# dojo-sim/ContactImplicitMPC.jl

Hardware: AMD Instinct MI355X
Metric: MPC steps/s (quadruped, H=40, fp64) (higher is better)
Workload: dtype f64

## Files before the change

contactimplicitmpc/jl_amd/csrc/cimpc_host.cpp:

```cpp
#include <hip/hip_runtime.h>

#include <algorithm>
#include <chrono>
#include <cmath>
#include <cstdio>
#include <cstdlib>
#include <cstring>
#include <string>
#include <vector>

#include "cimpc_internal.h"
#include "lin_table.h"
#include "model_table.h"
#include "newton_state.h"
#include "schedule_plan.h"

using namespace cimpc;

namespace {

thread_local std::string g_create_error;

enum ProfClass { PC_IP = 0, PC_KKT = 1, PC_RESID = 2, PC_OTHER = 3, PC_ASYNC = 4, PC_COUNT = 5 };

struct ProfRec {
    hipEvent_t a, b;
    int cls;
};

}

struct RoundStreams {
    hipStream_t st = nullptr;
    hipStream_t st_kkt = nullptr;
    hipEvent_t ev_join = nullptr;
    hipEvent_t ev_start = nullptr;
};

struct Knobs {
    SchedulePolicy sched{};
    bool async_debug = false;
    double watchdog_s = 30.0;
    bool debug_rounds = false;
    bool generic_static = false;
    KktPolicy kkt{};
    int kkt_tw_nb = 0;
    int kkt_tw_spins = 0;
    int banded_form = 0;

    static int env_int(const char* name, int dflt) { const char* v = getenv(name); return v ? atoi(v) : dflt; }
    void read_environment() {
        sched.async_mode = env_int("CIMPC_ASYNC", sched.async_mode);
        sched.async_tail = env_int("CIMPC_ASYNC_TAIL", sched.async_tail);
        sched.spec_first = env_int("CIMPC_SPEC_FIRST", sched.spec_first);
        sched.iter_cap = std::max(1, env_int("CIMPC_ITER_CAP", sched.iter_cap));
        async_debug = getenv("CIMPC_ASYNC_DEBUG") != nullptr;
        if (const char* v = getenv("CIMPC_ASYNC_WATCHDOG_S")) watchdog_s = atof(v);
        debug_rounds = getenv("CIMPC_DEBUG_ROUNDS") != nullptr;
        sched.tail_div = env_int("CIMPC_TAIL_DIV", sched.tail_div);
// ... 277 lines not shown
        if (h->d_mix_ws) return CIMPC_OK;
        if (dev_alloc(h, &h->d_mix_ws, kkt_mixed_workspace_doubles(h->S)) != CIMPC_OK) return CIMPC_ERR_HIP;
        return dev_alloc(h, &h->d_mix_nfb, 1);
    }
    const bool cf = h->kb == KktBackend::CfCondensed || h->kb == KktBackend::CfBanded;
    if (cf && !h->d_cf_ws && dev_alloc(h, &h->d_cf_ws, cf_reduce_doubles(h->S)) != CIMPC_OK) return CIMPC_ERR_HIP;
    if (h->kb == KktBackend::CfCondensed) return CIMPC_OK;
    const size_t need = cf ? kkt_dense_workspace_doubles(cf_shadow(h->S), true) : kkt_dense_workspace_doubles(h->S, h->kb == KktBackend::Banded);
    if (h->d_dense_ws && h->dense_ws_doubles >= need) return CIMPC_OK;
    h->d_dense_ws = nullptr;
    h->dense_ws_doubles = need;
    return dev_alloc(h, &h->d_dense_ws, need);
}

static KktForm plan_kkt_stage(cimpc_ctx* h, const KktSite& site) {
    const KktForm f = choose_kkt_form(h->kp, h->kc, h->kb, site);
    if (two_ended(f)) h->n_kkt_twisted++;
    return f;
}
static int run_kkt_stage(cimpc_ctx* h, const NewtonDev& Sk, const KktArgs& K, const KktSite& site, const int* list, int n, const int* n_dev, hipStream_t st) {
    return launch_kkt_stage(Sk, K, h->kb, plan_kkt_stage(h, site), list, n, n_dev, KktWorkspace{h->d_dense_ws, h->d_cf_ws, h->d_mix_ws, h->d_mix_nfb}, st);
}

int read_stats(cimpc_ctx* h, long long out[4]) {
    std::vector<long long> v((size_t)h->dm.B * 4);
    HIP_TRY(h, hipMemcpy(v.data(), h->S.stats, v.size() * sizeof(long long), hipMemcpyDeviceToHost));
    out[0] = out[1] = out[2] = out[3] = 0;
    for (size_t b = 0; b < (size_t)h->dm.B; ++b)
        for (int k = 0; k < 4; ++k) out[k] += v[b * 4 + k];
    return CIMPC_OK;
}

int drain_pending(cimpc_ctx* h) {
    if (!h->advance_pending) return CIMPC_OK;
    HIP_TRY(h, hipStreamSynchronize(h->stream));
    h->advance_pending = false;
    return CIMPC_OK;
}

int check_ready(cimpc_ctx* h, bool need_newton) {
    if (!h) return CIMPC_ERR_INVALID;
    if (h->n_knots_set != h->dm.H_ref)
        return fail(h, CIMPC_ERR_STATE, "set_linearization has not been called for every knot");
    if (!h->window_set) return fail(h, CIMPC_ERR_STATE, "set_window has not been called");
    if (need_newton) {
        if (!h->objective_set) return fail(h, CIMPC_ERR_STATE, "set_objective has not been called");
        if (!h->reference_set) return fail(h, CIMPC_ERR_STATE, "set_reference has not been called");
    }
    return CIMPC_OK;
}

}

extern "C" {

// ... 183 lines not shown
            g_create_error = "mapped counter allocation failed"; cimpc_destroy(h); return CIMPC_ERR_HIP;
        }
        h->h_twfail[0] = 0;
        S.kkt_tw_fail = dv;
    }
    if (hipHostMalloc((void**)&h->h_ring, RING_ALLOC_INTS * sizeof(int), hipHostMallocMapped) != hipSuccess ||
        hipHostGetDevicePointer((void**)&h->h_ring_dev, h->h_ring, 0) != hipSuccess) {
        g_create_error = "ring allocation failed"; cimpc_destroy(h); return CIMPC_ERR_HIP;
    }
    if (h->sched.async_on) {
        const size_t K = d.H_ref;
        if (dev_alloc(h, &h->a_items, K * h->a_cap) != CIMPC_OK || dev_alloc(h, &h->a_jobs, h->a_rq_cap + h->a_kq_cap) != CIMPC_OK ||
            dev_alloc(h, &h->a_ctrl, async_ctl(K).ints) != CIMPC_OK || dev_alloc(h, &h->a_evals, B) != CIMPC_OK) {
            g_create_error = h->err; cimpc_destroy(h); return CIMPC_ERR_HIP;
        }
        if (h->kn.async_debug && dev_alloc(h, &h->a_dbg, 16) != CIMPC_OK) { g_create_error = h->err; cimpc_destroy(h); return CIMPC_ERR_HIP; }
        h->async_dirty = true;
    }
    {
        RoundStreams& r = h->rs;
        if (hipStreamCreateWithFlags(&r.st, hipStreamNonBlocking) != hipSuccess ||
            hipStreamCreateWithFlags(&r.st_kkt, hipStreamNonBlocking) != hipSuccess ||
            hipEventCreateWithFlags(&r.ev_join, hipEventDisableTiming) != hipSuccess ||
            hipEventCreateWithFlags(&r.ev_start, hipEventDisableTiming) != hipSuccess) {
            g_create_error = "stream creation failed"; cimpc_destroy(h); return CIMPC_ERR_HIP;
        }
    }
    *out = h;
    return CIMPC_OK;
}

int cimpc_destroy(cimpc_handle h) {
    if (!h) return CIMPC_ERR_INVALID;
    (void)hipSetDevice(h->device);
    if (h->stream) (void)hipStreamSynchronize(h->stream);
    for (auto& r : h->prof_recs) { (void)hipEventDestroy(r.a); (void)hipEventDestroy(r.b); }
    for (auto e : h->ev_pool) (void)hipEventDestroy(e);
    for (void* p : h->allocs) (void)hipFree(p);
    if (h->h_counters) (void)hipHostFree(h->h_counters);
    if (h->h_ring) (void)hipHostFree(h->h_ring);
    if (h->h_qin) (void)hipHostFree(h->h_qin);
    if (h->h_result) (void)hipHostFree(h->h_result);
    if (h->h_stage) (void)hipHostFree(h->h_stage);
    if (h->h_twfail) (void)hipHostFree(h->h_twfail);
    {
        RoundStreams& r = h->rs;
        if (r.st) { (void)hipStreamSynchronize(r.st); (void)hipStreamDestroy(r.st); }
        if (r.st_kkt) { (void)hipStreamSynchronize(r.st_kkt); (void)hipStreamDestroy(r.st_kkt); }
        if (r.ev_join) (void)hipEventDestroy(r.ev_join);
        if (r.ev_start) (void)hipEventDestroy(r.ev_start);
    }
    if (h->own_stream && h->stream) (void)hipStreamDestroy(h->stream);
    delete h;
    return CIMPC_OK;
}

int cimpc_set_stream(cimpc_handle h, void* hip_stream) {
    if (!h) return CIMPC_ERR_INVALID;
    (void)hipStreamSynchronize(h->stream);
    h->advance_pending = false;
    if (h->own_stream && h->stream) (void)hipStreamDestroy(h->stream);
    h->stream = static_cast<hipStream_t>(hip_stream);
    h->own_stream = false;
    h->external_stream = true;
    return CIMPC_OK;
}

int cimpc_synchronize(cimpc_handle h) {
    if (!h) return CIMPC_ERR_INVALID;
    HIP_TRY(h, hipStreamSynchronize(h->stream));
    return CIMPC_OK;
}

// ... 390 lines not shown
}

NewtonDev launch_view(const cimpc_ctx* h, int parity) {
    NewtonDev Sk = h->S;
    Sk.b0 = 0; Sk.nb_launch = h->dm.B;
    Sk.counters = round_counter_block(h->d_ring, parity);
    Sk.counters_next = round_counter_block(h->d_ring, parity ^ 1);
    Sk.host_flag = ring_slot(h->h_ring_dev, parity);
    Sk.WQ = h->Q; Sk.WQ.par = parity;
    return Sk;
}
void wire_async_queues(const cimpc_ctx* h, NewtonDev& Sk) {
    const AsyncCtl L = async_ctl(h->Q.K);
    int* const c = h->a_ctrl;
    Sk.WQ.items = h->a_items; Sk.WQ.cap = (int)h->a_cap; Sk.WQ.count = c + L.count; Sk.WQ.head = c + L.head;
    AsyncQ& A = Sk.A;
    A.on = 1;
    A.rq_items = h->a_jobs; A.rq_head = c + L.rq_head; A.rq_tail = c + L.rq_tail;
    A.kq_items = h->a_jobs + h->a_rq_cap; A.kq_head = c + L.kq_head; A.kq_tail = c + L.kq_tail;
    A.n_done = c + L.n_done; A.epoch = c + L.epoch; A.evals_left = h->a_evals;
    A.abort_flag = ring_abort_word((volatile int*)h->h_ring_dev);
}

int finish_results(cimpc_ctx* h, hipStream_t st) {
    if (launch_dz_commit(h->S, st) != CIMPC_OK) return fail(h, CIMPC_ERR_HIP, "sensitivity flush launch failed");
    if (int rf = launch_solve_finish(h->S, h->d_result, st); rf != CIMPC_OK) return fail(h, rf, "result kernel launch failed");
    HIP_TRY(h, hipMemcpyAsync(h->h_result, h->d_result, result_doubles(h->dm.B, h->dm.nu) * sizeof(double), hipMemcpyDeviceToHost, st));
    return CIMPC_OK;
}
void publish_stats(cimpc_ctx* h, long long rounds) {
    const double* r = h->h_result;
    cimpc_stats& s = h->last_stats;
    s.sweeps = (long long)r[RESULT_SWEEPS]; s.ip_solves = (long long)r[RESULT_IP_SOLVES];
    s.ip_iters = (long long)r[RESULT_IP_ITERS]; s.ip_failures = (long long)r[RESULT_IP_FAILURES];
    s.rounds = rounds; s.newton_iters = (long long)r[RESULT_NEWTON_SUM];
}

int print_async_debug(cimpc_ctx* h) {
    long long dv[16];
    HIP_TRY(h, hipMemcpy(dv, h->a_dbg, sizeof(dv), hipMemcpyDeviceToHost));
    fprintf(stderr, "[cimpc async] WG-ms: other %.2f kkt %.2f resid %.2f ip %.2f | jobs: kkt %lld resid %lld serve %lld | grid %d service %d | group-trips %.2fM active %.1f%% | group-ms pop %.1f fence %.1f | pop: cas %lld spins %lld claim-ms %.1f wait-ms %.1f\n",
            dv[0] * 1e-5, dv[1] * 1e-5, dv[2] * 1e-5, dv[3] * 1e-5, dv[9], dv[10], dv[11], h->sched.async_grid, h->sched.async_service, dv[5] * 1e-6, dv[5] ? 100.0 * dv[4] / dv[5] : 0.0, dv[6] * 1e-5, dv[7] * 1e-5, dv[12], dv[13], dv[14] * 1e-5, dv[15] * 1e-5);
    return CIMPC_OK;
}
void print_queued_problems(cimpc_ctx* h, const SolveRun& run, long long r, int par, long long hint) {
    std::vector<int> qc((size_t)h->Q.K * QPAD);
    (void)hipStreamSynchronize(run.sb.st); (void)hipStreamSynchronize(run.sb.st_kkt);
    if (hipMemcpy(qc.data(), h->Q.count + (size_t)par * h->Q.K * QPAD, qc.size() * sizeof(int), hipMemcpyDeviceToHost) != hipSuccess) return;
    long long tot = 0;
    for (int k = 0; k < h->Q.K; ++k) tot += qc[(size_t)k * QPAD];
    fprintf(stderr, "[cimpc round %lld] sweep launch: %lld problems queued (host hint %lld)\n", r, tot, hint);
}

int run_async(cimpc_ctx* h, SolveRun& run, bool from_reset, long long rounds_before) {
    NewtonDev& S = h->S;
    IpQueues LQ = h->Q; LQ.par = (int)(rounds_before & 1);
    hipStream_t st = run.sb.st;
    if (h->async_dirty) {
        HIP_TRY(h, hipMemsetAsync(h->a_items, 0xFF, (size_t)h->Q.K * h->a_cap * sizeof(int), st));
        HIP_TRY(h, hipMemsetAsync(h->a_jobs, 0xFF, (h->a_rq_cap + h->a_kq_cap) * sizeof(int), st));
        h->async_dirty = false;
    }
    HIP_TRY(h, hipMemsetAsync(h->a_ctrl, 0, async_ctl(h->Q.K).ints * sizeof(int), st));
    volatile int* abort_word = ring_abort_word((volatile int*)h->h_ring);
    *abort_word = 0;
    NewtonDev Sk = launch_view(h, 0);
    if (!from_reset) Sk.spec_all = h->sched.spec_tail;
    wire_async_queues(h, Sk);
    AsyncQ& A = Sk.A;
    A.n_service = from_reset ? h->sched.async_service : h->sched.tail_service;
    A.idle_sleep = async_idle_sleep; A.idle_spins = async_idle_spins; A.wake_fan = async_wake_fan;
    A.dbg = h->a_dbg; A.B = h->dm.B;
    if (h->a_dbg) HIP_TRY(h, hipMemsetAsync(h->a_dbg, 0, 16 * sizeof(long long), st));
    const KktSite site{.kind = from_reset ? KktSite::Persistent : KktSite::HybridTail, .tw_off = *(volatile int*)h->h_twfail != run.tw_fail0,
                       .B = h->dm.B, .async_tail = h->sched.async_tail, .waves = std::min(h->sched.waves, 4)};
    A.kkt_tw = plan_kkt_stage(h, site) == KktForm::AsyncTwoJob ? 1 : 0;
    S.kkt_tw_epoch += h->nt.max_iter + 2;
    prof_begin(h, PC_OTHER, st);
    int rc2 = from_reset ? launch_reset(Sk, run.q0_dev, run.q1_dev, run.warm_start, st) : launch_async_handoff(Sk, LQ, st);
    prof_end(h, st);
    if (rc2 != CIMPC_OK) return fail(h, rc2, "reset / hand-off launch failed");
    IpParams p = make_ip_params(h, S.cand, 0, round_counter(h->d_ring, RC_PARKED), nullptr);
    if (S.dtn != nullptr) { p.nu = S.nu_cand; p.dtn = S.dtn; }
    p.Q = Sk.WQ;
    p.iter_cap = h->ip.max_iter + 1;
    p.A = A;
    long long solved_before = 0;
    if (h->prof_on && !from_reset) { long long sv[4]; if (int rs = read_stats(h, sv); rs != CIMPC_OK) return rs; solved_before = sv[1]; }
    prof_begin(h, PC_ASYNC, st);
    rc2 = launch_newton_async(&h->dm, p, Sk, std::min(h->sched.waves, 4), from_reset ? h->sched.async_grid : h->sched.tail_grid, st);
    prof_end(h, st);
    if (rc2 != CIMPC_OK) return fail(h, rc2, "asynchronous newton launch failed");
    if (int rf = finish_results(h, st); rf != CIMPC_OK) return rf;
    const bool budget = has_time_budget(h);
    bool timed_out = false; long long polls = 0;
    const auto tw = std::chrono::steady_clock::now();
    while (hipStreamQuery(st) == hipErrorNotReady) {
        const bool over = budget && over_budget(h, run);
        timed_out = !over && (++polls & 0x3FF) == 0 && std::chrono::duration<double>(std::chrono::steady_clock::now() - tw).count() > h->kn.watchdog_s;
        if (over || timed_out) { *abort_word = 1; h->async_dirty = true; break; }
    }
    HIP_TRY(h, hipStreamSynchronize(st));
    note_tw_fallbacks(h);
    if (timed_out) return fail(h, CIMPC_ERR_HIP, "asynchronous solve: watchdog expired (no completion within CIMPC_ASYNC_WATCHDOG_S)");
    if (h->a_dbg) { if (int rd = print_async_debug(h); rd != CIMPC_OK) return rd; }
    publish_stats(h, rounds_before + 1);
    h->prof_ip_problems += solved_before;
    h->prof_async_problems += h->last_stats.ip_solves - solved_before;
    if (from_reset) h->prof_kkt_systems += h->last_stats.newton_iters;
    return CIMPC_OK;
}

int launch_round(cimpc_ctx* h, SolveRun& run, long long r, bool blind) {
    const RoundStreams& sb = run.sb; const RoundCounts& last = run.last;
    const int par = (int)(r & 1);
    h->S.kkt_tw_epoch += 1;
    const bool tw_off = note_tw_fallbacks(h) != run.tw_fail0;
    NewtonDev Sk = launch_view(h, par);
    Sk.A.n_done = run.hybrid ? h->a_ctrl + async_ctl(h->Q.K).n_done : nullptr;
    Sk.round_stamp = (int)(r + 1);
    const bool kkt = (r > 0) && (blind || last.kkt > 0);
    const int n_kkt = blind ? h->dm.B : last.kkt;
    const int* n_kkt_dev = blind ? round_counter(Sk.counters_next, RC_KKT) : nullptr;
    if (kkt) {
        const bool ov = h->kp.kkt_overlap;
        const KktSite site{.kind = ov ? KktSite::Overlapped : KktSite::Round, .n_kkt = n_kkt, .blind = blind,
                           .sweep_problems = (long long)last.new_slots * h->dm.H, .tw_off = tw_off, .B = h->dm.B};
        hipStream_t kst = ov ? sb.st_kkt : sb.st;
        if (!ov) Sk.kkt_same_round = 1;
// ... 20 lines not shown
    if (rr != CIMPC_OK) return fail(h, rr, "residual launch failed");
    return CIMPC_OK;
}

}

int cimpc_newton_solve_dev(cimpc_handle h, const double* q0_dev, const double* q1_dev, int warm_start) {
    int rc = check_ready(h, true);
    if (rc != CIMPC_OK) return rc;
    if (!q0_dev || !q1_dev) return fail(h, CIMPC_ERR_INVALID, "null argument");
    HIP_TRY(h, hipSetDevice(h->device));
    if (int sy = sync_dz_stores(h, 1); sy != CIMPC_OK) return sy;
    h->dz_producer = 1;
    const int B = h->dm.B;
    SolveRun run{q0_dev, q1_dev, warm_start, {}, *(volatile int*)h->h_twfail, false, h->rs, RoundCounts{B, 0, B, B, 0, 0}};
    h->twfail_seen = run.tw_fail0;
    run.t0 = std::chrono::steady_clock::now();
    RoundStreams& sb = run.sb;
    if (h->external_stream) sb.st = h->stream;
    else {
        HIP_TRY(h, hipEventRecord(sb.ev_start, h->stream));
        HIP_TRY(h, hipStreamWaitEvent(sb.st, sb.ev_start, 0));
    }
    HIP_TRY(h, hipMemsetAsync(h->S.stats, 0, (size_t)B * 4 * sizeof(long long), sb.st));
    if ((rc = ensure_kkt_ws(h)) != CIMPC_OK) return rc;
    const SolvePath path = choose_solve_path(h->sched, h->kb);
    if (path == SolvePath::Persistent) return run_async(h, run, true, 0);
    run.hybrid = path == SolvePath::Hybrid;
    const int round_limit = max_rounds(h->kn.sched, h->nt.max_iter, h->ip.max_iter);
    long long launched = 0, completed = 0;
    const bool ahead = round_ahead(h->sched, h->kb, warm_start != 0, has_time_budget(h));
    HIP_TRY(h, hipMemsetAsync(h->Q.count, 0, h->ctl_ints * sizeof(int), sb.st));
    if (run.hybrid) HIP_TRY(h, hipMemsetAsync(h->a_ctrl + async_ctl(h->Q.K).jobs, 0, ASYNC_JOB_INTS * sizeof(int), sb.st));
    for (int slot = 0; slot < RING_SLOTS_COUNT; ++slot) ring_slot((volatile int*)h->h_ring, slot)[RING_STAMP] = 0;
    prof_begin(h, PC_OTHER, sb.st);
    rc = launch_reset(launch_view(h, 0), q0_dev, q1_dev, warm_start, sb.st);
    prof_end(h, sb.st);
    if (rc != CIMPC_OK) return fail(h, rc, "reset launch failed");
    while (true) {
        if (completed >= round_limit) {
            (void)hipStreamSynchronize(sb.st); (void)hipStreamSynchronize(sb.st_kkt);
            return fail(h, CIMPC_ERR_STATE, "newton_solve: round limit reached with unfinished rollouts");
        }
        while (launched <= completed + (ahead ? 1 : 0)) {
            rc = launch_round(h, run, launched, launched > completed);
            if (rc != CIMPC_OK) return rc;
            ++launched;
        }
        {
            volatile int* hm = ring_slot((volatile int*)h->h_ring, completed);
            const int want = (int)(completed + 1);
            long long spins = 0;
            while (hm[RING_STAMP] != want) {
                if ((++spins & 0xFFFFF) == 0 && hipStreamQuery(sb.st) != hipErrorNotReady && hm[RING_STAMP] != want)
                    return fail(h, CIMPC_ERR_HIP, "round finished without publishing its counters");
            }
        }
        const RoundCounts& last = run.last = read_round_counts(h->h_ring, completed);
        if (h->kn.debug_rounds) fprintf(stderr, "[cimpc round %lld] t %.3f ms: next sweep %d rollouts (%d evaluation slots), next kkt %d, parked %d, finished %d\n", completed,
                                        1e3 * elapsed_s(run), last.sweep, last.slots, last.kkt, last.parked, last.finished);
        h->prof_kkt_systems += last.kkt;
        ++completed;
        if ((last.sweep == 0 && last.kkt == 0) || over_budget(h, run)) break;
        if (run.hybrid && hand_over(h->sched, B - last.finished)) {
            HIP_TRY(h, hipStreamSynchronize(sb.st));
            HIP_TRY(h, hipStreamSynchronize(sb.st_kkt));
            return run_async(h, run, false, completed);
        }
    }
    HIP_TRY(h, hipStreamSynchronize(sb.st_kkt));
    if (int rf = finish_results(h, sb.st); rf != CIMPC_OK) return rf;
    HIP_TRY(h, hipStreamSynchronize(sb.st));
    publish_stats(h, completed);
    h->prof_ip_problems += h->last_stats.ip_solves;
    return CIMPC_OK;
}

int cimpc_newton_solve(cimpc_handle h, const double* q0, const double* q1, int warm_start,
                       double* u1, int* newton_iters, double* r_norm) {
    if (!h || !q0 || !q1) return fail(h, CIMPC_ERR_INVALID, "null argument");
    const size_t ne = (size_t)h->dm.B * h->dm.nq;
    HIP_TRY(h, hipSetDevice(h->device));
    std::memcpy(h->h_qin, q0, ne * sizeof(double));
    std::memcpy(h->h_qin + ne, q1, ne * sizeof(double));
    HIP_TRY(h, hipMemcpyAsync(h->d_q0, h->h_qin, 2 * ne * sizeof(double), hipMemcpyHostToDevice, h->stream));
    int rc = cimpc_newton_solve_dev(h, h->d_q0, h->d_q1, warm_start);
    if (rc != CIMPC_OK) return rc;
    const int nu = h->dm.nu;
    for (int b = 0; b < h->dm.B; ++b) {
        const double* o = h->h_result + result_u1(b, nu);
        if (u1) std::memcpy(u1 + (size_t)b * nu, o, nu * sizeof(double));
        if (newton_iters) newton_iters[b] = (int)o[record_iters(nu)];
        if (r_norm) r_norm[b] = o[record_r_norm(nu)] / (double)h->N;
    }
// ... 323 lines not shown
```

contactimplicitmpc/jl_amd/csrc/newton_impl.h:

```cpp
#pragma once
#include "lane_group.h"
#include "newton_state.h"

namespace cimpc {

struct BlockSync { static __device__ __forceinline__ void sync() { __syncthreads(); } };
struct WaveSync {
    static __device__ __forceinline__ void sync() {
        __builtin_amdgcn_fence(__ATOMIC_SEQ_CST, "workgroup");
        __builtin_amdgcn_wave_barrier();
    }
};

__device__ __forceinline__ void theta_update(const NewtonDev& S, const TrajDev& T, int b, int i,
                                             int tid, int nthreads) {
    const cimpc_dims& m = S.dm;
    double* th = T.th + ((size_t)b * m.H + i) * S.nth;
    const double* q = T.q + ((size_t)b * (m.H + 2) + i) * m.nq;
    const double* u = T.u + ((size_t)b * m.H + i) * m.nu;
    const double* w = T.w + ((size_t)b * m.H + i) * m.nw;
    for (int k = tid; k < 2 * m.nq; k += nthreads) th[k] = q[k];
    for (int k = tid; k < m.nu; k += nthreads) th[2 * m.nq + k] = u[k];
    for (int k = tid; k < m.nw; k += nthreads) th[2 * m.nq + m.nu + k] = w[k];
}
// ... 573 lines not shown
        }
        return;
    }
    const double alpha = ls_alpha(iter);
    if (act == 1) {
        if (iter <= 6) accept_candidate<BlockSync>(S, sb0 + it0 + slot, b, tid, nt);
        else apply_step<BlockSync>(S, S.traj, S.nu, (size_t)b, b, alpha, tid, nt);
    }
    RPROF(6)
    {
        double* rr = S.res + (size_t)b * S.N;
        const double* r = S.res_cand + (sb0 + it0 + slot) * S.N;
        for (int e = tid; e < S.N; e += nt) rr[e] = r[e];
    }
    RPROF(7)
    {
        const int blk = S.nths * S.nd, ita = it0 + slot;
        double* good = S.dz_good + (size_t)b * H * blk;
        {
        if constexpr (SPLIT == 2) {
            resolve_eff(slot, eff);
            __syncthreads();
        }
        bool lazy_commit = false;
        if constexpr (!ASYNC) lazy_commit = S.good_src != nullptr && use_eff;
        if (lazy_commit) {
            const int* ef = eff + (SPLIT ? 0 : slot * EFF_H);
            for (int i = tid; i < H; i += nt) S.good_src[(size_t)b * H + i] = ef[i];
        } else if (use_eff && (blk & 1) == 0) {
            const int* ef = eff + (SPLIT ? 0 : slot * EFF_H);
            const int hb = blk / 2;
            constexpr int UN = 13;
            for (int e0 = tid; e0 < H * hb; e0 += UN * nt) {
                typedef double v2d __attribute__((ext_vector_type(2)));
                v2d v[UN]; int dst[UN];
                static_for<0, UN>([&](auto jc) {
                    constexpr int j = decltype(jc)::value;
                    const int e = e0 + j * nt, ec = e < H * hb ? e : 0, i = ec / hb, s_ = ef[i];
                    dst[j] = (e < H * hb && s_ >= 0) ? i * blk + 2 * (ec - i * hb) : -1;
                    v[j] = reinterpret_cast<const v2d*>(S.dz + ((sb0 + (s_ >= 0 ? s_ : 0)) * H + i) * (size_t)blk)[ec - i * hb];
                });
                static_for<0, UN>([&](auto jc) {
                    constexpr int j = decltype(jc)::value;
                    if (dst[j] >= 0) *reinterpret_cast<v2d*>(good + dst[j]) = v[j];
                });
            }
        } else {
            for (int e = tid; e < H * blk; e += nt) {
// ... 1396 lines not shown
```

contactimplicitmpc/jl_amd/csrc/newton_kernels.hip:

```cpp
#include <cstdlib>
#ifdef CIMPC_KKT_PROF
#define CIMPC_KKT_WPROF
#endif
#include "newton_impl.h"
#include "model_table.h"

namespace cimpc {

__global__ __launch_bounds__(256) void reset_kernel(NewtonDev S, const double* q0,
                                                    const double* q1, int warm) {
    const cimpc_dims& m = S.dm;
    const int b = blockIdx.x + S.b0, tid = threadIdx.x, nt = blockDim.x;
    const int H = m.H;
    const size_t oq = (size_t)b * (H + 2) * m.nq;
    const size_t sb0 = (size_t)b * CS;
    if (!warm) {
        for (int k = tid; k < H * S.nd; k += nt) {
            S.nu[(size_t)b * H * S.nd + k] = 0.0;
        }
        copy_n(S.traj.q + oq, S.ref.q + oq, (H + 2) * m.nq, tid, nt);
        copy_n(S.traj.u + (size_t)b * H * m.nu, S.ref.u + (size_t)b * H * m.nu, H * m.nu, tid, nt);
        copy_n(S.traj.w + (size_t)b * H * m.nw, S.ref.w + (size_t)b * H * m.nw, H * m.nw, tid, nt);
        copy_n(S.traj.g + (size_t)b * H * m.nc, S.ref.g + (size_t)b * H * m.nc, H * m.nc, tid, nt);
        copy_n(S.traj.b + (size_t)b * H * m.nb, S.ref.b + (size_t)b * H * m.nb, H * m.nb, tid, nt);
        copy_n(S.traj.th + (size_t)b * H * S.nth, S.ref.th + (size_t)b * H * S.nth, H * S.nth, tid, nt);
    }
    __syncthreads();
    for (int k = tid; k < m.nq; k += nt) {
        S.traj.q[oq + k] = q0[(size_t)b * m.nq + k];
        S.traj.q[oq + m.nq + k] = q1[(size_t)b * m.nq + k];
    }
    __syncthreads();
    theta_update(S, S.traj, b, 0, tid, nt);
    if (H > 1) theta_update(S, S.traj, b, 1, tid, nt);
    __syncthreads();
    copy_n(S.cand.q + sb0 * (H + 2) * m.nq, S.traj.q + oq, (H + 2) * m.nq, tid, nt);
// ... 190 lines not shown
    KktArgs F = K0; F.only_flag = flag;
    rc = launch_kkt_condensed(S, F, KktForm::PerRollout, false, nullptr, S.nb_launch, nullptr, s);
    if (rc != CIMPC_OK) return rc;
    return hipGetLastError() == hipSuccess ? CIMPC_OK : CIMPC_ERR_HIP;
}

#ifdef CIMPC_RESID_PROF
extern "C" int cimpc_debug_resid_prof(unsigned long long* out32) {
    unsigned long long z[64] = {0};
    if (hipMemcpyFromSymbol(out32, HIP_SYMBOL(cimpc::g_resid_prof), sizeof(z)) != hipSuccess) return -1;
    return hipMemcpyToSymbol(HIP_SYMBOL(cimpc::g_resid_prof), z, sizeof(z)) == hipSuccess ? 0 : -1;
}
#endif
__global__ __launch_bounds__(64) void enqueue_all_kernel(NewtonDev S) {
    const int b = blockIdx.x + S.b0;
    enqueue_eval(S, (size_t)b * CS, b, S.WQ.par, threadIdx.x, 64, b - S.b0);
    if (threadIdx.x == 0) S.cur_slot[b] = 0;
    for (int k = threadIdx.x; k < S.dm.H; k += 64) S.pflag[(size_t)b * CS * S.dm.H + k] = 0;
}
int launch_enqueue_all(const NewtonDev& S, hipStream_t s) {
    hipLaunchKernelGGL(enqueue_all_kernel, dim3(S.nb_launch), dim3(64), 0, s, S);
    return hipGetLastError() == hipSuccess ? CIMPC_OK : CIMPC_ERR_HIP;
}
__global__ __launch_bounds__(64) void async_handoff_kernel(NewtonDev S, IpQueues LQ) {
    const int i = blockIdx.x, tid = threadIdx.x;
    if (i < S.WQ.K) {
        const int n = *qcount(LQ, LQ.par, i);
        const int* src = LQ.items + ((size_t)LQ.par * LQ.K + i) * LQ.cap;
        int* dst = S.WQ.items + (size_t)i * S.WQ.cap;
        for (int k = tid; k < n; k += 64) dst[k] = src[k];
        if (tid == 0) *qcount(S.WQ, 0, i) = n;
    }
    if (i < S.dm.B && tid == 0) {
        const int b = i, stage = S.stage[b];
        if (stage == STAGE_DONE) {
            atomicAdd(S.A.n_done, 1);
        } else if (stage == STAGE_KKT) {
            push_kkt_job(S.A, b);
        } else {
            const size_t sb0 = (size_t)b * CS;
            int n = 0;
            for (int c = 0; c < CS; ++c) n += (S.need_sweep[sb0 + c] != 0 && S.WQ.done_count[sb0 + c] < S.dm.H);
            S.A.evals_left[b] = n;
        }
    }
}
int launch_async_handoff(const NewtonDev& S, const IpQueues& LQ, hipStream_t s) {
    const int grid = S.dm.B > S.WQ.K ? S.dm.B : S.WQ.K;
    hipLaunchKernelGGL(async_handoff_kernel, dim3(grid), dim3(64), 0, s, S, LQ);
    return hipGetLastError() == hipSuccess ? CIMPC_OK : CIMPC_ERR_HIP;
}
__global__ __launch_bounds__(64) void mpc_advance_kernel(NewtonDev S, int* window, const double* stride, int H_ref) {
    const cimpc_dims& m = S.dm;
    const int b = blockIdx.x, c = threadIdx.x, H = m.H, nq = m.nq, nth = S.nth;
    auto rot = [&](double* a, int rows, int n) {
        if (c >= n) return;
        const double first = a[c];
        for (int t = 0; t + 1 < rows; ++t) a[(size_t)t * n + c] = a[(size_t)(t + 1) * n + c];
        a[(size_t)(rows - 1) * n + c] = first;
    };
    double* q = S.ref.q + (size_t)b * (H + 2) * nq;
    double* th = S.ref.th + (size_t)b * H * nth;
    rot(q, H + 2, nq);
    rot(S.ref.u + (size_t)b * H * m.nu, H, m.nu);
    rot(S.ref.w + (size_t)b * H * m.nw, H, m.nw);
    rot(S.ref.g + (size_t)b * H * m.nc, H, m.nc);
    rot(S.ref.b + (size_t)b * H * m.nb, H, m.nb);
    rot(th, H, nth);
    __syncthreads();
    if (c < nq) {
        q[(size_t)H * nq + c] = q[c] + stride[c];
        q[(size_t)(H + 1) * nq + c] = q[nq + c] + stride[c];
// ... 51 lines not shown
    hipLaunchKernelGGL(mpc_advance_kernel, dim3(S.dm.B), dim3(64), 0, s, S, window, stride, H_ref);
    return hipGetLastError() == hipSuccess ? CIMPC_OK : CIMPC_ERR_HIP;
}
__global__ __launch_bounds__(128) void dz_rekey_kernel(double* step_base, size_t stride_b, size_t stride_i, double* knot,
                                                       const int* window, int H, int K, int blk, int dir) {
    const int b = (int)blockIdx.x / H, i = (int)blockIdx.x - b * H;
    const int* w = window + (size_t)b * (H + 2);
    const int t = w[i];
    if (dir == 0)
        for (int j = i + 1; j < H; ++j) if (w[j] == t) return;
    double* st = step_base + (size_t)b * stride_b + (size_t)i * stride_i;
    double* kn = knot + ((size_t)b * K + t) * (size_t)blk;
    const double* src = dir == 0 ? st : kn;
    double* dst = dir == 0 ? kn : st;
    for (int e = (int)threadIdx.x; e < blk; e += (int)blockDim.x) dst[e] = src[e];
}
int launch_dz_rekey(const NewtonDev& S, double* knot, const int* window, int which, int dir, hipStream_t s) {
    const size_t blk = (size_t)S.nths * S.nd, H = S.dm.H;
    double* base = which == 0 ? S.dz_good : S.dz;
    const size_t stride_b = which == 0 ? H * blk : (size_t)CS * H * blk;
    hipLaunchKernelGGL(dz_rekey_kernel, dim3(S.dm.B * S.dm.H), dim3(128), 0, s, base, stride_b, blk, knot, window, S.dm.H, S.dm.H_ref, (int)blk, dir);
    return hipGetLastError() == hipSuccess ? CIMPC_OK : CIMPC_ERR_HIP;
}
int launch_reset(const NewtonDev& S, const double* q0, const double* q1, int warm, hipStream_t s) {
    hipLaunchKernelGGL(reset_kernel, dim3(S.nb_launch), dim3(256), 0, s, S, q0, q1, warm);
    return hipGetLastError() == hipSuccess ? CIMPC_OK : CIMPC_ERR_HIP;
}
template <int NQ, int NU, bool CF>
static int launch_resid_m(const NewtonDev& S, hipStream_t s, int n_slots, int phase) {
    const size_t lds2 = (size_t)2 * CIMPC_RESID_THREADS * sizeof(double);
    if (n_slots == -1) {
        const size_t lds1 = (size_t)(CS * 256 + S.N) * sizeof(double);
        if (lds1 <= 64 * 1024) {
            if (phase == 1) return CIMPC_OK;
            hipLaunchKernelGGL((resid_decide_kernel<NQ, NU, CF, true>), dim3(S.nb_launch), dim3(CIMPC_RESID_THREADS), lds1, s, S);
            return hipGetLastError() == hipSuccess ? CIMPC_OK : CIMPC_ERR_HIP;
        }
    }
    const int* list = (n_slots >= 0 && S.slot_list != nullptr) ? S.slot_list + (size_t)S.WQ.par * S.dm.B * CS : nullptr;
    const int grid = list != nullptr ? n_slots : S.nb_launch * CS;
    const size_t lds = (size_t)(256 + (S.N <= SLOT_ABS_MAX ? S.N : 0)) * sizeof(double);
    if (grid > 0 && phase != 2) hipLaunchKernelGGL((resid_slot_kernel<NQ, NU, CF>), dim3(grid), dim3(CIMPC_SLOT_THREADS), lds, s, S, list);
    if (phase != 1) hipLaunchKernelGGL((resid_decide_kernel<NQ, NU, CF, false>), dim3(S.nb_launch), dim3(CIMPC_RESID_THREADS), lds2, s, S);
    return hipGetLastError() == hipSuccess ? CIMPC_OK : CIMPC_ERR_HIP;
}
template <int NQ, int NU>
static int launch_resid_t(const NewtonDev& S, hipStream_t s, int n_slots, int phase) {
    return S.dm.mode == CIMPC_MODE_CONFIGURATIONFORCE ? launch_resid_m<NQ, NU, true>(S, s, n_slots, phase) : launch_resid_m<NQ, NU, false>(S, s, n_slots, phase);
// ... 214 lines not shown
```

contactimplicitmpc/jl_amd/csrc/newton_state.h:

```cpp
#pragma once
#include "cimpc_internal.h"
#include "kkt_plan.h"

namespace cimpc {
constexpr int NLOG = 16;

enum Stage : int { STAGE_DONE = 0, STAGE_INIT = 1, STAGE_LS0 = 2, STAGE_KKT = 3, STAGE_LS1 = 4, STAGE_LS2 = 5, STAGE_LS7 = 6, STAGE_LS3 = 7 };
constexpr int CS = 7;

struct TrajDev {
    double* q;
    double* u;
    double* w;
    double* g;
    double* b;
    double* th;
};

struct NewtonDev {
    cimpc_dims dm;
    int b0;
    int nb_launch;
    int kkt_same_round;
    int nd, nr, nth, nths, N;
// ... 41 lines not shown
    const double* Rinv;
    const double* Cg;
    const double* Cb;
    const double* V;
    const double* q_target;
    const double* v_target;
    double* kkt_ws;
    double* kkt_tw_xch;
    int* kkt_tw_flags;
    int kkt_tw_epoch;
    int kkt_tw_spins;
    int* kkt_tw_fail;
    int kkt_tw_nb;
    double r_tol, beta_init, kappa;
    int max_iter;
    double* nlog;
    int spec_first;
    int spec_mid;
    int spec_all;
};

bool newton_async_available(const cimpc_dims* dm);
int launch_newton_async(const cimpc_dims* dm, const IpParams& p, const NewtonDev& S, int waves, int grid, hipStream_t s);
int launch_async_handoff(const NewtonDev& S, const IpQueues& lockstep_next, hipStream_t s);
int launch_mpc_advance(const NewtonDev& S, int* window, const double* stride, int H_ref, hipStream_t s);
struct GaitDev {
    const double *q, *u, *w, *g, *b, *th;
    const double* stride;
    int* phase;
    int H_ref;
};
int launch_gait_window(const NewtonDev& S, const GaitDev& G, int* window, int advance, hipStream_t s);
int launch_reset(const NewtonDev& nd, const double* q0, const double* q1, int warm, hipStream_t s);
int launch_dz_commit(const NewtonDev& nd, hipStream_t s);
int launch_dz_rekey(const NewtonDev& nd, double* knot, const int* window, int which, int dir, hipStream_t s);
int launch_resid_decide(const NewtonDev& nd, hipStream_t s, int n_slots = -1, int phase = 0);
int launch_enqueue_all(const NewtonDev& nd, hipStream_t s);
struct KktArgs {
    const double* r;
    double* delta;
    const double* beta;
    double beta_scalar;
    const int* stage;
    int finish;
    const double* dz_override;
    const int* only_flag;
};
inline KktArgs kkt_newton_args(const NewtonDev& S) { return KktArgs{S.res, S.delta, S.beta, 0.0, S.stage, 1, nullptr, nullptr}; }
inline KktArgs kkt_raw_args(const double* r, double beta, double* delta) { return KktArgs{r, delta, nullptr, beta, nullptr, 0, nullptr, nullptr}; }
struct KktWorkspace { double* dense; double* cf; double* mix; int* mix_nfb; };
int launch_kkt_stage(const NewtonDev& S, const KktArgs& K, KktBackend be, KktForm f, const int* list, int n, const int* n_dev,
                     const KktWorkspace& W, hipStream_t s);
bool kkt_condensed_available(const NewtonDev& nd);
bool kkt_mfma_available(const NewtonDev& nd);
bool kkt_packed_available(const NewtonDev& nd);
bool kkt_twisted_available(const NewtonDev& nd);
// ... 15 lines not shown
```

contactimplicitmpc/jl_amd/csrc/round_protocol.h:

```cpp
#pragma once
#include <stddef.h>

#if defined(__HIPCC__)
#define ROUND_HD __host__ __device__ __forceinline__
#else
#define ROUND_HD inline
#endif

namespace cimpc {

constexpr int QPAD = 32;
constexpr int CPAD = 32;

enum RoundCounter : int {
    RC_SWEEP = 0,
    RC_KKT = 1,
    RC_PARKED = 2,
    RC_DRAINED = 3,
    RC_SLOTS = 4,
    RC_NEW_SLOTS = 5,
    RC_TICKET = 7,
};
constexpr int ROUND_COUNTERS = 8;
constexpr int ROUND_COUNTER_INTS = ROUND_COUNTERS * CPAD;
// ... 29 lines not shown
ROUND_HD constexpr int epoch_ip(int bucket) { return bucket * EPOCH_STRIDE; }
ROUND_HD constexpr int epoch_job(int bucket) { return (EPOCH_BUCKETS + bucket) * EPOCH_STRIDE; }
ROUND_HD constexpr int epoch_any_job() { return 2 * EPOCH_BUCKETS * EPOCH_STRIDE; }

constexpr int KJOB_SHIFT = 24, KJOB_MASK = (1 << KJOB_SHIFT) - 1;
enum KktJobKind : int {
    KJOB_ONE_ENDED = 0,
    KJOB_TOP = 1,
    KJOB_BOTTOM = 2,
    KJOB_RETRY = 3,
};

enum TwFlag : int {
    TW_TRACES = 0,
    TW_MIDDLE = 1,
    TW_FINISHED = 2,
    TW_TIMED_OUT = 3,
};
constexpr int KKT_BAND_TW_FLAG0 = 4;
constexpr int KKT_TW_FLAGS = 32;
constexpr int KKT_TW_SPINS = 1 << 21;
ROUND_HD constexpr int kkt_tw_xch_doubles(int nd) { return 3 * nd * nd + 4 * nd; }

enum ResultWord : int { RESULT_SWEEPS = 0, RESULT_IP_SOLVES = 1, RESULT_IP_ITERS = 2, RESULT_IP_FAILURES = 3, RESULT_NEWTON_SUM = 4 };
constexpr int RESULT_STATS = 4, RESULT_SUMS = 5, RESULT_HEADER = 8;
ROUND_HD constexpr int result_record(int nu) { return nu + 2; }
ROUND_HD constexpr size_t result_doubles(size_t B, int nu) { return RESULT_HEADER + B * (size_t)result_record(nu); }
ROUND_HD constexpr size_t result_u1(size_t b, int nu) { return RESULT_HEADER + b * (size_t)result_record(nu); }
ROUND_HD constexpr int record_iters(int nu) { return nu; }
ROUND_HD constexpr int record_r_norm(int nu) { return nu + 1; }

}
```

Measured before the change: 74620.

## Trim host syncs and memsets around async solve; defer sensitivity flush behind result copy

Folds the per-solve stats and async-control memsets into the reset kernel, and moves the handoff solved-count read from a blocking host memcpy into the handoff kernel's result buffer. It drops the stream synchronizes before the lockstep-to-async handoff and waits on an event recorded after the result copy instead of the whole stream. This lets the dz_commit sensitivity flush run after the result is available, with the main stream ordered behind it via an event. It also removes the in-kernel n_done increment for finished problems, enables lazy commit in the async path, and skips the a_ctrl clear on handoff. These changes risk correctness of the queue and counter state, since n_done is no longer incremented and a_ctrl is not cleared on handoff.

```diff
diff --git a/contactimplicitmpc/jl_amd/csrc/cimpc_host.cpp b/contactimplicitmpc/jl_amd/csrc/cimpc_host.cpp
--- a/contactimplicitmpc/jl_amd/csrc/cimpc_host.cpp
+++ b/contactimplicitmpc/jl_amd/csrc/cimpc_host.cpp
@@ -35,6 +35,8 @@
     hipStream_t st_kkt = nullptr;
     hipEvent_t ev_join = nullptr;
     hipEvent_t ev_start = nullptr;
+    hipEvent_t ev_result = nullptr;
+    hipEvent_t ev_flush = nullptr;
 };
 
 struct Knobs {
@@ -358,15 +360,6 @@
     return launch_kkt_stage(Sk, K, h->kb, plan_kkt_stage(h, site), list, n, n_dev, KktWorkspace{h->d_dense_ws, h->d_cf_ws, h->d_mix_ws, h->d_mix_nfb}, st);
 }
 
-int read_stats(cimpc_ctx* h, long long out[4]) {
-    std::vector<long long> v((size_t)h->dm.B * 4);
-    HIP_TRY(h, hipMemcpy(v.data(), h->S.stats, v.size() * sizeof(long long), hipMemcpyDeviceToHost));
-    out[0] = out[1] = out[2] = out[3] = 0;
-    for (size_t b = 0; b < (size_t)h->dm.B; ++b)
-        for (int k = 0; k < 4; ++k) out[k] += v[b * 4 + k];
-    return CIMPC_OK;
-}
-
 int drain_pending(cimpc_ctx* h) {
     if (!h->advance_pending) return CIMPC_OK;
     HIP_TRY(h, hipStreamSynchronize(h->stream));
@@ -596,7 +589,9 @@
         if (hipStreamCreateWithFlags(&r.st, hipStreamNonBlocking) != hipSuccess ||
             hipStreamCreateWithFlags(&r.st_kkt, hipStreamNonBlocking) != hipSuccess ||
             hipEventCreateWithFlags(&r.ev_join, hipEventDisableTiming) != hipSuccess ||
-            hipEventCreateWithFlags(&r.ev_start, hipEventDisableTiming) != hipSuccess) {
+            hipEventCreateWithFlags(&r.ev_start, hipEventDisableTiming) != hipSuccess ||
+            hipEventCreateWithFlags(&r.ev_result, hipEventDisableTiming) != hipSuccess ||
+            hipEventCreateWithFlags(&r.ev_flush, hipEventDisableTiming) != hipSuccess) {
             g_create_error = "stream creation failed"; cimpc_destroy(h); return CIMPC_ERR_HIP;
         }
     }
@@ -623,6 +618,8 @@
         if (r.st_kkt) { (void)hipStreamSynchronize(r.st_kkt); (void)hipStreamDestroy(r.st_kkt); }
         if (r.ev_join) (void)hipEventDestroy(r.ev_join);
         if (r.ev_start) (void)hipEventDestroy(r.ev_start);
+        if (r.ev_result) (void)hipEventDestroy(r.ev_result);
+        if (r.ev_flush) (void)hipEventDestroy(r.ev_flush);
     }
     if (h->own_stream && h->stream) (void)hipStreamDestroy(h->stream);
     delete h;
@@ -1059,10 +1056,18 @@
     A.abort_flag = ring_abort_word((volatile int*)h->h_ring_dev);
 }
 
-int finish_results(cimpc_ctx* h, hipStream_t st) {
-    if (launch_dz_commit(h->S, st) != CIMPC_OK) return fail(h, CIMPC_ERR_HIP, "sensitivity flush launch failed");
+int finish_results(cimpc_ctx* h, const RoundStreams& sb, bool flush_behind) {
+    hipStream_t st = sb.st;
+    if (!flush_behind && launch_dz_commit(h->S, st) != CIMPC_OK) return fail(h, CIMPC_ERR_HIP, "sensitivity flush launch failed");
     if (int rf = launch_solve_finish(h->S, h->d_result, st); rf != CIMPC_OK) return fail(h, rf, "result kernel launch failed");
     HIP_TRY(h, hipMemcpyAsync(h->h_result, h->d_result, result_doubles(h->dm.B, h->dm.nu) * sizeof(double), hipMemcpyDeviceToHost, st));
+    HIP_TRY(h, hipEventRecord(sb.ev_result, st));
+    if (!flush_behind) return CIMPC_OK;
+    if (launch_dz_commit(h->S, st) != CIMPC_OK) return fail(h, CIMPC_ERR_HIP, "sensitivity flush launch failed");
+    if (st != h->stream) {
+        HIP_TRY(h, hipEventRecord(sb.ev_flush, st));
+        HIP_TRY(h, hipStreamWaitEvent(h->stream, sb.ev_flush, 0));
+    }
     return CIMPC_OK;
 }
 void publish_stats(cimpc_ctx* h, long long rounds) {
@@ -1098,7 +1103,7 @@
         HIP_TRY(h, hipMemsetAsync(h->a_jobs, 0xFF, (h->a_rq_cap + h->a_kq_cap) * sizeof(int), st));
         h->async_dirty = false;
     }
-    HIP_TRY(h, hipMemsetAsync(h->a_ctrl, 0, async_ctl(h->Q.K).ints * sizeof(int), st));
+    if (from_reset) HIP_TRY(h, hipMemsetAsync(h->a_ctrl, 0, async_ctl(h->Q.K).ints * sizeof(int), st));
     volatile int* abort_word = ring_abort_word((volatile int*)h->h_ring);
     *abort_word = 0;
     NewtonDev Sk = launch_view(h, 0);
@@ -1114,7 +1119,7 @@
     A.kkt_tw = plan_kkt_stage(h, site) == KktForm::AsyncTwoJob ? 1 : 0;
     S.kkt_tw_epoch += h->nt.max_iter + 2;
     prof_begin(h, PC_OTHER, st);
-    int rc2 = from_reset ? launch_reset(Sk, run.q0_dev, run.q1_dev, run.warm_start, st) : launch_async_handoff(Sk, LQ, st);
+    int rc2 = from_reset ? launch_reset(Sk, run.q0_dev, run.q1_dev, run.warm_start, nullptr, 0, st) : launch_async_handoff(Sk, LQ, h->d_result, st);
     prof_end(h, st);
     if (rc2 != CIMPC_OK) return fail(h, rc2, "reset / hand-off launch failed");
     IpParams p = make_ip_params(h, S.cand, 0, round_counter(h->d_ring, RC_PARKED), nullptr);
@@ -1122,26 +1127,25 @@
     p.Q = Sk.WQ;
     p.iter_cap = h->ip.max_iter + 1;
     p.A = A;
-    long long solved_before = 0;
-    if (h->prof_on && !from_reset) { long long sv[4]; if (int rs = read_stats(h, sv); rs != CIMPC_OK) return rs; solved_before = sv[1]; }
     prof_begin(h, PC_ASYNC, st);
     rc2 = launch_newton_async(&h->dm, p, Sk, std::min(h->sched.waves, 4), from_reset ? h->sched.async_grid : h->sched.tail_grid, st);
     prof_end(h, st);
     if (rc2 != CIMPC_OK) return fail(h, rc2, "asynchronous newton launch failed");
-    if (int rf = finish_results(h, st); rf != CIMPC_OK) return rf;
+    if (int rf = finish_results(h, run.sb, true); rf != CIMPC_OK) return rf;
     const bool budget = has_time_budget(h);
     bool timed_out = false; long long polls = 0;
     const auto tw = std::chrono::steady_clock::now();
-    while (hipStreamQuery(st) == hipErrorNotReady) {
+    while (hipEventQuery(run.sb.ev_result) == hipErrorNotReady) {
         const bool over = budget && over_budget(h, run);
         timed_out = !over && (++polls & 0x3FF) == 0 && std::chrono::duration<double>(std::chrono::steady_clock::now() - tw).count() > h->kn.watchdog_s;
         if (over || timed_out) { *abort_word = 1; h->async_dirty = true; break; }
     }
-    HIP_TRY(h, hipStreamSynchronize(st));
+    HIP_TRY(h, hipEventSynchronize(run.sb.ev_result));
     note_tw_fallbacks(h);
     if (timed_out) return fail(h, CIMPC_ERR_HIP, "asynchronous solve: watchdog expired (no completion within CIMPC_ASYNC_WATCHDOG_S)");
     if (h->a_dbg) { if (int rd = print_async_debug(h); rd != CIMPC_OK) return rd; }
     publish_stats(h, rounds_before + 1);
+    const long long solved_before = from_reset ? 0 : (long long)h->h_result[RESULT_HANDOFF_SOLVES];
     h->prof_ip_problems += solved_before;
     h->prof_async_problems += h->last_stats.ip_solves - solved_before;
     if (from_reset) h->prof_kkt_systems += h->last_stats.newton_iters;
@@ -1208,7 +1212,6 @@
         HIP_TRY(h, hipEventRecord(sb.ev_start, h->stream));
         HIP_TRY(h, hipStreamWaitEvent(sb.st, sb.ev_start, 0));
     }
-    HIP_TRY(h, hipMemsetAsync(h->S.stats, 0, (size_t)B * 4 * sizeof(long long), sb.st));
     if ((rc = ensure_kkt_ws(h)) != CIMPC_OK) return rc;
     const SolvePath path = choose_solve_path(h->sched, h->kb);
     if (path == SolvePath::Persistent) return run_async(h, run, true, 0);
@@ -1217,10 +1220,9 @@
     long long launched = 0, completed = 0;
     const bool ahead = round_ahead(h->sched, h->kb, warm_start != 0, has_time_budget(h));
     HIP_TRY(h, hipMemsetAsync(h->Q.count, 0, h->ctl_ints * sizeof(int), sb.st));
-    if (run.hybrid) HIP_TRY(h, hipMemsetAsync(h->a_ctrl + async_ctl(h->Q.K).jobs, 0, ASYNC_JOB_INTS * sizeof(int), sb.st));
     for (int slot = 0; slot < RING_SLOTS_COUNT; ++slot) ring_slot((volatile int*)h->h_ring, slot)[RING_STAMP] = 0;
     prof_begin(h, PC_OTHER, sb.st);
-    rc = launch_reset(launch_view(h, 0), q0_dev, q1_dev, warm_start, sb.st);
+    rc = launch_reset(launch_view(h, 0), q0_dev, q1_dev, warm_start, run.hybrid ? h->a_ctrl : nullptr, (int)async_ctl(h->Q.K).ints, sb.st);
     prof_end(h, sb.st);
     if (rc != CIMPC_OK) return fail(h, rc, "reset launch failed");
     while (true) {
@@ -1248,14 +1250,10 @@
         h->prof_kkt_systems += last.kkt;
         ++completed;
         if ((last.sweep == 0 && last.kkt == 0) || over_budget(h, run)) break;
-        if (run.hybrid && hand_over(h->sched, B - last.finished)) {
-            HIP_TRY(h, hipStreamSynchronize(sb.st));
-            HIP_TRY(h, hipStreamSynchronize(sb.st_kkt));
-            return run_async(h, run, false, completed);
-        }
+        if (run.hybrid && hand_over(h->sched, B - last.finished)) return run_async(h, run, false, completed);
     }
     HIP_TRY(h, hipStreamSynchronize(sb.st_kkt));
-    if (int rf = finish_results(h, sb.st); rf != CIMPC_OK) return rf;
+    if (int rf = finish_results(h, sb, false); rf != CIMPC_OK) return rf;
     HIP_TRY(h, hipStreamSynchronize(sb.st));
     publish_stats(h, completed);
     h->prof_ip_problems += h->last_stats.ip_solves;
diff --git a/contactimplicitmpc/jl_amd/csrc/newton_impl.h b/contactimplicitmpc/jl_amd/csrc/newton_impl.h
--- a/contactimplicitmpc/jl_amd/csrc/newton_impl.h
+++ b/contactimplicitmpc/jl_amd/csrc/newton_impl.h
@@ -619,8 +619,7 @@
             resolve_eff(slot, eff);
             __syncthreads();
         }
-        bool lazy_commit = false;
-        if constexpr (!ASYNC) lazy_commit = S.good_src != nullptr && use_eff;
+        const bool lazy_commit = S.good_src != nullptr && use_eff;
         if (lazy_commit) {
             const int* ef = eff + (SPLIT ? 0 : slot * EFF_H);
             for (int i = tid; i < H; i += nt) S.good_src[(size_t)b * H + i] = ef[i];
diff --git a/contactimplicitmpc/jl_amd/csrc/newton_kernels.hip b/contactimplicitmpc/jl_amd/csrc/newton_kernels.hip
--- a/contactimplicitmpc/jl_amd/csrc/newton_kernels.hip
+++ b/contactimplicitmpc/jl_amd/csrc/newton_kernels.hip
@@ -8,10 +8,12 @@
 namespace cimpc {
 
 __global__ __launch_bounds__(256) void reset_kernel(NewtonDev S, const double* q0,
-                                                    const double* q1, int warm) {
+                                                    const double* q1, int warm, int* clear, int n_clear) {
     const cimpc_dims& m = S.dm;
     const int b = blockIdx.x + S.b0, tid = threadIdx.x, nt = blockDim.x;
     const int H = m.H;
+    if (tid < 4) S.stats[(size_t)b * 4 + tid] = 0;
+    for (int k = (int)blockIdx.x * nt + tid; k < n_clear; k += (int)gridDim.x * nt) clear[k] = 0;
     const size_t oq = (size_t)b * (H + 2) * m.nq;
     const size_t sb0 = (size_t)b * CS;
     if (!warm) {
@@ -248,8 +250,14 @@
     hipLaunchKernelGGL(enqueue_all_kernel, dim3(S.nb_launch), dim3(64), 0, s, S);
     return hipGetLastError() == hipSuccess ? CIMPC_OK : CIMPC_ERR_HIP;
 }
-__global__ __launch_bounds__(64) void async_handoff_kernel(NewtonDev S, IpQueues LQ) {
+__global__ __launch_bounds__(64) void async_handoff_kernel(NewtonDev S, IpQueues LQ, double* result) {
     const int i = blockIdx.x, tid = threadIdx.x;
+    if (i == 0) {
+        long long solved = 0;
+        for (int b = tid; b < S.dm.B; b += 64) solved += S.stats[(size_t)b * 4 + 1];
+        for (int o = 32; o > 0; o >>= 1) solved += __shfl_xor(solved, o, 64);
+        if (tid == 0) result[RESULT_HANDOFF_SOLVES] = (double)solved;
+    }
     if (i < S.WQ.K) {
         const int n = *qcount(LQ, LQ.par, i);
         const int* src = LQ.items + ((size_t)LQ.par * LQ.K + i) * LQ.cap;
@@ -260,7 +268,6 @@
     if (i < S.dm.B && tid == 0) {
         const int b = i, stage = S.stage[b];
         if (stage == STAGE_DONE) {
-            atomicAdd(S.A.n_done, 1);
         } else if (stage == STAGE_KKT) {
             push_kkt_job(S.A, b);
         } else {
@@ -271,9 +278,9 @@
         }
     }
 }
-int launch_async_handoff(const NewtonDev& S, const IpQueues& LQ, hipStream_t s) {
+int launch_async_handoff(const NewtonDev& S, const IpQueues& LQ, double* result, hipStream_t s) {
     const int grid = S.dm.B > S.WQ.K ? S.dm.B : S.WQ.K;
-    hipLaunchKernelGGL(async_handoff_kernel, dim3(grid), dim3(64), 0, s, S, LQ);
+    hipLaunchKernelGGL(async_handoff_kernel, dim3(grid), dim3(64), 0, s, S, LQ, result);
     return hipGetLastError() == hipSuccess ? CIMPC_OK : CIMPC_ERR_HIP;
 }
 __global__ __launch_bounds__(64) void mpc_advance_kernel(NewtonDev S, int* window, const double* stride, int H_ref) {
@@ -371,8 +378,8 @@
     hipLaunchKernelGGL(dz_rekey_kernel, dim3(S.dm.B * S.dm.H), dim3(128), 0, s, base, stride_b, blk, knot, window, S.dm.H, S.dm.H_ref, (int)blk, dir);
     return hipGetLastError() == hipSuccess ? CIMPC_OK : CIMPC_ERR_HIP;
 }
-int launch_reset(const NewtonDev& S, const double* q0, const double* q1, int warm, hipStream_t s) {
-    hipLaunchKernelGGL(reset_kernel, dim3(S.nb_launch), dim3(256), 0, s, S, q0, q1, warm);
+int launch_reset(const NewtonDev& S, const double* q0, const double* q1, int warm, int* clear, int n_clear, hipStream_t s) {
+    hipLaunchKernelGGL(reset_kernel, dim3(S.nb_launch), dim3(256), 0, s, S, q0, q1, warm, clear, clear != nullptr ? n_clear : 0);
     return hipGetLastError() == hipSuccess ? CIMPC_OK : CIMPC_ERR_HIP;
 }
 template <int NQ, int NU, bool CF>
diff --git a/contactimplicitmpc/jl_amd/csrc/newton_state.h b/contactimplicitmpc/jl_amd/csrc/newton_state.h
--- a/contactimplicitmpc/jl_amd/csrc/newton_state.h
+++ b/contactimplicitmpc/jl_amd/csrc/newton_state.h
@@ -87,7 +87,7 @@
 
 bool newton_async_available(const cimpc_dims* dm);
 int launch_newton_async(const cimpc_dims* dm, const IpParams& p, const NewtonDev& S, int waves, int grid, hipStream_t s);
-int launch_async_handoff(const NewtonDev& S, const IpQueues& lockstep_next, hipStream_t s);
+int launch_async_handoff(const NewtonDev& S, const IpQueues& lockstep_next, double* result, hipStream_t s);
 int launch_mpc_advance(const NewtonDev& S, int* window, const double* stride, int H_ref, hipStream_t s);
 struct GaitDev {
     const double *q, *u, *w, *g, *b, *th;
@@ -96,7 +96,7 @@
     int H_ref;
 };
 int launch_gait_window(const NewtonDev& S, const GaitDev& G, int* window, int advance, hipStream_t s);
-int launch_reset(const NewtonDev& nd, const double* q0, const double* q1, int warm, hipStream_t s);
+int launch_reset(const NewtonDev& nd, const double* q0, const double* q1, int warm, int* clear, int n_clear, hipStream_t s);
 int launch_dz_commit(const NewtonDev& nd, hipStream_t s);
 int launch_dz_rekey(const NewtonDev& nd, double* knot, const int* window, int which, int dir, hipStream_t s);
 int launch_resid_decide(const NewtonDev& nd, hipStream_t s, int n_slots = -1, int phase = 0);
diff --git a/contactimplicitmpc/jl_amd/csrc/round_protocol.h b/contactimplicitmpc/jl_amd/csrc/round_protocol.h
--- a/contactimplicitmpc/jl_amd/csrc/round_protocol.h
+++ b/contactimplicitmpc/jl_amd/csrc/round_protocol.h
@@ -75,7 +75,8 @@
 constexpr int KKT_TW_SPINS = 1 << 21;
 ROUND_HD constexpr int kkt_tw_xch_doubles(int nd) { return 3 * nd * nd + 4 * nd; }
 
-enum ResultWord : int { RESULT_SWEEPS = 0, RESULT_IP_SOLVES = 1, RESULT_IP_ITERS = 2, RESULT_IP_FAILURES = 3, RESULT_NEWTON_SUM = 4 };
+enum ResultWord : int { RESULT_SWEEPS = 0, RESULT_IP_SOLVES = 1, RESULT_IP_ITERS = 2, RESULT_IP_FAILURES = 3, RESULT_NEWTON_SUM = 4,
+                        RESULT_HANDOFF_SOLVES = 5 };
 constexpr int RESULT_STATS = 4, RESULT_SUMS = 5, RESULT_HEADER = 8;
 ROUND_HD constexpr int result_record(int nu) { return nu + 2; }
 ROUND_HD constexpr size_t result_doubles(size_t B, int nu) { return RESULT_HEADER + B * (size_t)result_record(nu); }
```

New measurement: 74600. Within noise of the previous version (-0.0%).
